# Tongji-MIC-Lab/TDVC

Hardware: AMD Instinct MI355X
Metric: 1080p P-frames/sec (encode + reconstruct, lambda=2048 config) (higher is better)
Workload: dtype f16; 1 GPU; 1x 1920x1080 (padded 1088x1920) 7-frame synthetic GOP (seed 1234), batch 1, P-frames coded in GOP order; gop=7, batch=1, parallelism=gop-sharded x1, weights=closed-form filler (no checkpoint ships)

## Files before the change

include/tdvc_hip.h:

```cpp
#ifndef TDVC_HIP_H
#define TDVC_HIP_H

#include <stdint.h>

#ifdef __cplusplus
extern "C" {
#endif

#define TDVC_OK 0
#define TDVC_EINVAL (-1)
#define TDVC_ENOSUP (-2)

typedef struct {
  void* p;
  int32_t N, H, W, C;
  int64_t sn;
  int32_t sp;
  int32_t dtype;
} tdvc_fmap;

enum { TDVC_F16 = 0, TDVC_F32 = 1 };
enum { TDVC_ACT_NONE = 0, TDVC_ACT_RELU = 1, TDVC_ACT_LRELU = 2, TDVC_ACT_CLAMP01 = 3, TDVC_ACT_SIGMOID = 4 };
enum { TDVC_GDN_NONE = 0, TDVC_GDN_FWD = 1, TDVC_GDN_INV = 2 };
enum { TDVC_OUT_NHWC = 0,
       TDVC_OUT_SHUFFLE2 = 1,
       TDVC_OUT_NCHW_F32 = 2 };

#define TDVC_MAX_TAPS 49

typedef struct {
  tdvc_fmap x;
  tdvc_fmap y;
  const void* w;
  const float* bias;
  int32_t cout;
  int32_t ntaps;
  int8_t tap_dy[TDVC_MAX_TAPS], tap_dx[TDVC_MAX_TAPS];
  int32_t kh, kw, stride, pad;
  int32_t ck;
  int32_t square_input;
  int32_t gdn;
  tdvc_fmap aux;
  int32_t act; float slope;
  int32_t round_before_act;
  tdvc_fmap res;
  tdvc_fmap res2;
  int32_t out_mode;
  int32_t s2d;
  int32_t bcast_T;
  float bcast_slope;
  float* chan_sum;
  tdvc_fmap flow;
} tdvc_conv_desc;

int tdvc_abi_version(void);
const char* tdvc_last_error(void);
int tdvc_prepare_device(void);
const char* tdvc_last_conv_kernel(void);

int tdvc_set_predicate(const int* flag);
int tdvc_last_launch_predicated(void);
#define TDVC_MAX_PREDICATE_IMAGES 4
int tdvc_set_predicate_images(const int* flags, int n);
int tdvc_frame_changed(const tdvc_fmap* cur, tdvc_fmap* cache, int* flag, void* stream);
int tdvc_frames_changed(const tdvc_fmap* cur, tdvc_fmap* cache, int* flags, unsigned force_mask, void* stream);


int tdvc_conv_plan(int cin, int kh, int kw, int stride);
int64_t tdvc_conv_packed_bytes(int cout, int cin, int ntaps, int ck);
int tdvc_pack_conv_weights(const float* w_oihw, int cout, int cin_real, int cin, int kh, int kw,
                           int ntaps, const int8_t* tap_dy, const int8_t* tap_dx, int ck, uint16_t* dst);
int tdvc_conv2d(const tdvc_conv_desc* d, void* stream);
int tdvc_conv_chan_sum_rows(const tdvc_conv_desc* d);
int tdvc_conv_flow_supported(const tdvc_conv_desc* d);
const char* tdvc_conv_select(const tdvc_conv_desc* d);
int tdvc_conv2d_f32(const tdvc_conv_desc* d, void* stream);

typedef struct {
  tdvc_fmap x, y;
  const void* w;
  const float* bias;
  int32_t act1; float slope1;
  int32_t act2; float slope2;
  int32_t add_input;
  tdvc_fmap res2;
} tdvc_conv_pair_desc;
int64_t tdvc_conv_pair_packed_bytes(void);
int tdvc_pack_conv_pair_weights(const float* w1_oihw, const float* w2_oihw, uint16_t* dst);
int tdvc_conv_pair_supported(const tdvc_conv_pair_desc* d);
int tdvc_conv_pair(const tdvc_conv_pair_desc* d, void* stream);

typedef struct {
  tdvc_fmap s, a, y;
  int32_t nslices;
  int32_t slice_stride;
  const void* wt;
  const float* bias_t;
  const void* w3;
  const float* bias3;
  float slope;
} tdvc_lf_tail_desc;
int tdvc_lf_tail_supported(const tdvc_lf_tail_desc* d);
int tdvc_lf_tail(const tdvc_lf_tail_desc* d, void* stream);

typedef struct {
  tdvc_fmap x, om, y;
  const void* w;
  const float* bias;
  int32_t groups;
  int32_t act; float slope; int32_t round_before_act;
  void* x_planar;
} tdvc_dcn_desc;
int tdvc_dcn_fused(const tdvc_dcn_desc* d, void* stream);

int tdvc_dcn_v2_forward_f32(const float* input, const float* weight, const float* bias,
                            const float* offset, const float* mask, float* output,
                            int B, int C, int H, int W, int Cout,
                            int kh, int kw, int sh, int sw, int ph, int pw, int dh, int dw,
                            int deformable_group, void* stream);
int tdvc_dcn_v2_backward_f32(const float* input, const float* weight, const float* bias,
                             const float* offset, const float* mask, const float* grad_output,
                             float* grad_input, float* grad_offset, float* grad_mask,
                             float* grad_weight, float* grad_bias, float* columns,
                             int B, int C, int H, int W, int Cout,
                             int kh, int kw, int sh, int sw, int ph, int pw, int dh, int dw,
                             int deformable_group, void* stream);

int tdvc_nchw_to_fmap(const float* src, int C, const tdvc_fmap* y, void* stream);
int tdvc_fmap_to_nchw(const tdvc_fmap* x, int C, float* dst, void* stream);
int tdvc_scale_act_res(const tdvc_fmap* a, const float* gate, int act, float slope,
                       const tdvc_fmap* r, float r_sign, const tdvc_fmap* y, const tdvc_fmap* y2, void* stream);
int tdvc_scale_act_res3(const tdvc_fmap* a, const float* gate, int act, float slope, const tdvc_fmap* r, float r_sign,
                        const tdvc_fmap* y, const tdvc_fmap* b, float b_sign, const tdvc_fmap* y3, void* stream);
int tdvc_add_flow(const tdvc_fmap* off, const tdvc_fmap* flow, void* stream);
int tdvc_bcast_add_act(const tdvc_fmap* x, const tdvc_fmap* b, int T, float slope, void* stream);

int tdvc_channel_sum(const tdvc_fmap* x, float* partial, int nblocks, void* stream);
int tdvc_se_gate(const float* partial, int nblocks, float inv_count, int N, int C, int Cmid,
                 const float* w1, const float* b1, const float* w2, const float* b2,
                 float* gate, void* stream);

int tdvc_upsample2x(const tdvc_fmap* x, const tdvc_fmap* y, void* stream);
int tdvc_avgpool2(const tdvc_fmap* x, const tdvc_fmap* y, void* stream);
int tdvc_avgpool2_pyramid(const tdvc_fmap* xa, const tdvc_fmap* xb, const tdvc_fmap* ya, const tdvc_fmap* yb, void* stream);
int tdvc_spynet_level_input(const tdvc_fmap* ref, const tdvc_fmap* supp, const tdvc_fmap* flow_lo,
                            const tdvc_fmap* flow_up, const tdvc_fmap* cat8, void* stream);
int tdvc_resize_bilinear(const tdvc_fmap* x, const tdvc_fmap* y, const float* chscale, void* stream);

int64_t tdvc_avgpool_k_work_floats(int N, int hp, int wp, int C, int scale);
int tdvc_avgpool_k(const tdvc_fmap* x, int scale, float* pooled, int hp, int wp, float* work, int64_t work_floats, void* stream);
int tdvc_patch_match(const float* pin, const float* pref, int N, int hp, int wp, int C,
                     int32_t* idx, void* stream);
int tdvc_match_gather(const tdvc_fmap* fin, const tdvc_fmap* fref, const int32_t* idx, int scale,
                      int hp, int wp, const tdvc_fmap* cat, void* stream);

int tdvc_eb_forward(const tdvc_fmap* z, const float* params, const tdvc_fmap* noise,
                    const tdvc_fmap* z_hat, double* bits_out, float* partial, int partial_cap, void* stream);
int tdvc_gc_forward(const tdvc_fmap* y, const tdvc_fmap* gp, const tdvc_fmap* noise,
                    double* bits_out, float* partial, int partial_cap, void* stream);
int tdvc_quantize(const tdvc_fmap* y, const tdvc_fmap* noise, const tdvc_fmap* y_hat, void* stream);

int64_t tdvc_rans_encode(const int32_t* symbols, const int32_t* indexes, int64_t n,
                         const int32_t* cdfs, int32_t cdf_stride, const int32_t* cdf_sizes,
                         const int32_t* offsets, uint8_t* out, int64_t cap);
int tdvc_rans_decode(const uint8_t* data, int64_t nbytes, const int32_t* indexes, int64_t n,
                     const int32_t* cdfs, int32_t cdf_stride, const int32_t* cdf_sizes,
                     const int32_t* offsets, int32_t* symbols_out);

void* tdvc_rans_decoder_create(const uint8_t* data, int64_t nbytes);
int tdvc_rans_decoder_decode(void* handle, const int32_t* indexes, int64_t n, const int32_t* cdfs,
                             int32_t cdf_stride, const int32_t* cdf_sizes, const int32_t* offsets,
                             int32_t* symbols_out);
void tdvc_rans_decoder_destroy(void* handle);

int64_t tdvc_rans_encode_lanes(const int32_t* symbols, const int32_t* indexes, int64_t npos, int M, int L,
                               const int32_t* cdfs, int32_t cdf_stride, const int32_t* cdf_sizes,
                               const int32_t* offsets, uint8_t* out, int64_t cap);
int tdvc_rans_decode_lanes(const uint8_t* data, int64_t nbytes, const int32_t* indexes, int64_t npos, int M,
                           const int32_t* cdfs, int32_t cdf_stride, const int32_t* cdf_sizes,
                           const int32_t* offsets, int32_t* symbols_out);

int tdvc_pmf_to_quantized_cdf(const float* pmf, int n, int precision, int32_t* cdf_out);

int tdvc_ar_gather_batch(const tdvc_fmap* y_hat, const tdvc_fmap* params, const int32_t* pos, int npos,
                         const tdvc_fmap* x1, const tdvc_fmap* pc, void* stream);
int tdvc_ar_quantize_batch(const tdvc_fmap* y, const tdvc_fmap* gp, const int32_t* pos, int npos, const float* scale_table, int ntable,
                           const int32_t* symbols_in, const tdvc_fmap* y_hat, int32_t* symbols, int32_t* indexes, int64_t cbase, void* stream);
int tdvc_ar_indexes_batch(const tdvc_fmap* gp, const int32_t* pos, int npos, int B, const float* scale_table, int ntable,
                          int M, int H, int W, int32_t* indexes, int64_t cbase, void* stream);
typedef struct tdvc_cdf_tables {
  const int32_t *cdfs, *sizes, *offsets;
  int32_t stride, ncdfs;
} tdvc_cdf_tables;
typedef struct tdvc_cdf_tables_dev {
  const uint16_t* cdf16;
  const int32_t *starts, *sizes, *offsets;
  int32_t n16, ncdfs;
} tdvc_cdf_tables_dev;
typedef struct tdvc_ar_loop {
  tdvc_fmap y_hat, params;
  tdvc_fmap x1, pc, gp;
  const tdvc_conv_desc* convs;
  int32_t nconvs;
  const int32_t* pos_dev;
  const int32_t* step_sizes;
  int32_t nsteps;
  const float* scale_table;
  int32_t ntable;
  int32_t *idx_dev, *sym_dev;
} tdvc_ar_loop;
int tdvc_ar_wavefront_batch(const tdvc_ar_loop* loop, const tdvc_fmap* y, const uint8_t* const* data, const int64_t* nbytes,
                            const tdvc_cdf_tables* tables, void* stream);
int tdvc_ar_decode_serial_batch(const tdvc_ar_loop* loop, const uint8_t* const* data, const int64_t* nbytes, const tdvc_cdf_tables* tables,
                                void* stream);
int64_t tdvc_ar_lanes_state_bytes(int L);
int64_t tdvc_ar_lanes_batch_layout(const int64_t* nbytes, int B, int L, uint32_t* table_out);
int tdvc_ar_lanes_init_batch(const uint8_t* streams_dev, int64_t stream_bytes, const uint32_t* table_dev, int B, int L, uint32_t* state_dev, void* stream);
int tdvc_ar_decode_lanes_step_batch(const tdvc_fmap* gp, const int32_t* pos, int npos, const float* scale_table, int ntable,
                                    const uint8_t* streams_dev, int64_t stream_bytes, const uint32_t* table_dev, int L,
                                    const tdvc_cdf_tables_dev* tables, uint32_t* state_dev, const tdvc_fmap* y_hat,
                                    int32_t* symbols, int32_t* indexes, int64_t cbase, void* stream);
int tdvc_ar_wavefront_lanes_batch(const tdvc_ar_loop* loop, const uint8_t* const* data, const int64_t* nbytes, uint8_t* stream_dev,
                                  int64_t stream_cap, uint32_t* state_dev, const tdvc_cdf_tables_dev* tables, int32_t* bad_image, void* stream);
int64_t tdvc_ar_encode_lanes_scratch_words(int64_t npos, int M, int L);
int64_t tdvc_ar_encode_lanes_out_bytes(int64_t npos, int M, int L);
typedef struct tdvc_lanes_enc {
  const int32_t *symbols, *indexes;
  int32_t B, H, W, M;
// ... 118 lines not shown
```

tdvc_amd/_lib.py:

```python
from __future__ import annotations

import ctypes as C
import os

_HERE = os.path.dirname(os.path.abspath(__file__))
LIB_PATH = os.path.join(_HERE, "libtdvc_hip.so")

MAX_TAPS = 49
F16, F32 = 0, 1
ACT_NONE, ACT_RELU, ACT_LRELU, ACT_CLAMP01, ACT_SIGMOID = 0, 1, 2, 3, 4
GDN_NONE, GDN_FWD, GDN_INV = 0, 1, 2
OUT_NHWC, OUT_SHUFFLE2, OUT_NCHW_F32 = 0, 1, 2


class FMapDesc(C.Structure):
    _fields_ = [("p", C.c_void_p), ("N", C.c_int32), ("H", C.c_int32), ("W", C.c_int32), ("C", C.c_int32),
                ("sn", C.c_int64), ("sp", C.c_int32), ("dtype", C.c_int32)]


class ConvDesc(C.Structure):
    _fields_ = [("x", FMapDesc), ("y", FMapDesc), ("w", C.c_void_p), ("bias", C.c_void_p),
                ("cout", C.c_int32), ("ntaps", C.c_int32),
                ("tap_dy", C.c_int8 * MAX_TAPS), ("tap_dx", C.c_int8 * MAX_TAPS),
                ("kh", C.c_int32), ("kw", C.c_int32), ("stride", C.c_int32), ("pad", C.c_int32),
                ("ck", C.c_int32), ("square_input", C.c_int32), ("gdn", C.c_int32),
                ("aux", FMapDesc), ("act", C.c_int32), ("slope", C.c_float),
                ("round_before_act", C.c_int32), ("res", FMapDesc), ("res2", FMapDesc), ("out_mode", C.c_int32), ("s2d", C.c_int32),
                ("bcast_T", C.c_int32), ("bcast_slope", C.c_float), ("chan_sum", C.c_void_p), ("flow", FMapDesc)]


class DcnDesc(C.Structure):
    _fields_ = [("x", FMapDesc), ("om", FMapDesc), ("y", FMapDesc), ("w", C.c_void_p), ("bias", C.c_void_p),
                ("groups", C.c_int32), ("act", C.c_int32), ("slope", C.c_float), ("round_before_act", C.c_int32), ("x_planar", C.c_void_p)]


class ConvPairDesc(C.Structure):
    _fields_ = [("x", FMapDesc), ("y", FMapDesc), ("w", C.c_void_p), ("bias", C.c_void_p), ("act1", C.c_int32), ("slope1", C.c_float),
                ("act2", C.c_int32), ("slope2", C.c_float), ("add_input", C.c_int32), ("res2", FMapDesc)]


class LfTailDesc(C.Structure):
    _fields_ = [("s", FMapDesc), ("a", FMapDesc), ("y", FMapDesc), ("nslices", C.c_int32), ("slice_stride", C.c_int32),
                ("wt", C.c_void_p), ("bias_t", C.c_void_p), ("w3", C.c_void_p), ("bias3", C.c_void_p), ("slope", C.c_float)]


class WgradReduceJob(C.Structure):
    _fields_ = [("work", C.c_void_p), ("bwork", C.c_void_p), ("row_off", C.c_void_p), ("chan_off", C.c_void_p), ("tap_off", C.c_void_p),
                ("bias_index", C.c_void_p), ("dw", C.c_void_p), ("db", C.c_void_p), ("scale", C.c_float),
                ("nworkers", C.c_int32), ("cow", C.c_int32), ("ciw", C.c_int32), ("ntaps", C.c_int32), ("cout", C.c_int32), ("cin", C.c_int32),
                ("wblocks", C.c_int32), ("nblocks", C.c_int32)]


_P = C.c_void_p
_FM = C.POINTER(FMapDesc)


class CdfTablesDesc(C.Structure):
    _fields_ = [("cdfs", _P), ("sizes", _P), ("offsets", _P), ("stride", C.c_int32), ("ncdfs", C.c_int32)]


class CdfTablesDevDesc(C.Structure):
    _fields_ = [("cdf16", _P), ("starts", _P), ("sizes", _P), ("offsets", _P), ("n16", C.c_int32), ("ncdfs", C.c_int32)]


class ArLoopDesc(C.Structure):
    _fields_ = [("y_hat", FMapDesc), ("params", FMapDesc), ("x1", FMapDesc), ("pc", FMapDesc), ("gp", FMapDesc),
                ("convs", C.POINTER(ConvDesc)), ("nconvs", C.c_int32), ("pos_dev", _P), ("step_sizes", _P), ("nsteps", C.c_int32),
                ("scale_table", _P), ("ntable", C.c_int32), ("idx_dev", _P), ("sym_dev", _P)]


class LanesEncDesc(C.Structure):
    _fields_ = [("symbols", _P), ("indexes", _P), ("B", C.c_int32), ("H", C.c_int32), ("W", C.c_int32), ("M", C.c_int32), ("pos", _P),
                ("npos", C.c_int32), ("L", C.c_int32), ("scratch", _P), ("lane_words", C.c_int64), ("scratch_cap_words", C.c_int64),
                ("out", _P), ("out_stride", C.c_int64), ("out_cap", C.c_int64), ("info", _P)]


_LOOP, _CDF, _CDFD, _ENC = C.POINTER(ArLoopDesc), C.POINTER(CdfTablesDesc), C.POINTER(CdfTablesDevDesc), C.POINTER(LanesEncDesc)
_i, _f, _i64 = C.c_int, C.c_float, C.c_int64

SIGNATURES = {
    "tdvc_abi_version": (_i, []),
    "tdvc_conv_chan_sum_rows": (_i, [C.POINTER(ConvDesc)]),
    "tdvc_conv_select": (C.c_char_p, [C.POINTER(ConvDesc)]),
    "tdvc_conv_flow_supported": (_i, [C.POINTER(ConvDesc)]),
    "tdvc_scale_act_res3": (_i, [_FM, _P, _i, _f, _FM, _f, _FM, _FM, _f, _FM, _P]),
    "tdvc_avgpool2_pyramid": (_i, [_FM, _FM, _FM, _FM, _P]),
    "tdvc_last_error": (C.c_char_p, []),
    "tdvc_last_conv_kernel": (C.c_char_p, []),
    "tdvc_prepare_device": (_i, []),
    "tdvc_set_predicate": (_i, [_P]),
    "tdvc_set_predicate_images": (_i, [_P, _i]),
    "tdvc_last_launch_predicated": (_i, []),
    "tdvc_frame_changed": (_i, [_FM, _FM, _P, _P]),
    "tdvc_frames_changed": (_i, [_FM, _FM, _P, C.c_uint, _P]),
    "tdvc_conv_plan": (_i, [_i, _i, _i, _i]),
    "tdvc_conv_packed_bytes": (_i64, [_i, _i, _i, _i]),
    "tdvc_pack_conv_weights": (_i, [_P, _i, _i, _i, _i, _i, _i, _P, _P, _i, _P]),
    "tdvc_conv2d": (_i, [C.POINTER(ConvDesc), _P]),
    "tdvc_conv2d_f32": (_i, [C.POINTER(ConvDesc), _P]),
    "tdvc_pack_conv_weights_indexed": (_i, [_P] * 7 + [_i] * 4 + [_P, _P]),
    "tdvc_pack_conv_weights_indexed_f32": (_i, [_P] * 7 + [_i] * 4 + [_P, _P]),
    "tdvc_pack_job_blocks": (_i64, [_i, _i, _i, _i]),
    "tdvc_pack_conv_weights_batch": (_i, [_P, _P, _i, _i, _P]),
    "tdvc_act_backward": (_i, [_FM, _FM, _FM, _i, _f, _FM, _P]),
    "tdvc_pixel_unshuffle": (_i, [_FM, _FM, _P]),
    "tdvc_bias_grad_work_floats": (_i64, [_i, _i]),
    "tdvc_bias_grad": (_i, [_FM, _i, _P, _f, _P, _P, _i64, _P]),
    "tdvc_copy_cast": (_i, [_FM, _FM, _P]),
    "tdvc_clamp01_backward": (_i, [_FM, _FM, _P]),
    "tdvc_gate_backward_work_floats": (_i64, [_i, _i]),
    "tdvc_gate_backward": (_i, [_FM, _FM, _P, _FM, _P, _P, _i64, _P]),
    "tdvc_se_gate_backward": (_i, [_P, _i, _f, _i, _i, _i] + [_P] * 6 + [_f] + [_P] * 6),
    "tdvc_bcast_channel_add": (_i, [_FM, _P, _f, _P]),
    "tdvc_add_flow_backward": (_i, [_FM, _FM, _P]),
    "tdvc_bcast_add_act_backward": (_i, [_FM, _FM, _FM, _f, _P]),
    "tdvc_upsample2x_backward": (_i, [_FM, _FM, _P]),
    "tdvc_resize_bilinear_backward": (_i, [_FM, _FM, _P, _P]),
    "tdvc_spynet_level_input_backward": (_i, [_FM, _FM, _FM, _FM, _FM, _P]),
    "tdvc_sigmoid_f32": (_i, [_P, _P, _i64, _P]),
    "tdvc_sigmoid_backward_f32": (_i, [_P, _P, _i64, _P]),
    "tdvc_axpy_f32": (_i, [_P, _P, _f, _i64, _P]),
    "tdvc_match_gather_backward": (_i, [_FM, _FM, _P, _i, _i, _i, _FM, _FM, _FM, _P]),
    "tdvc_eb_backward": (_i, [_FM, _P, _FM, _f, _FM, _P, _P]),
    "tdvc_eb_pack": (_i, [_P, _P, _P, _i, _P]),
    "tdvc_eb_param_chain": (_i, [_P, _P, _P, _f, _i, _P]),
    "tdvc_eb_aux": (_i, [_P, _P, _f, _P, _P, _i, _P]),
    "tdvc_gc_backward": (_i, [_FM, _FM, _FM, _f, _FM, _FM, _P]),
    "tdvc_dcn_columns": (_i, [_FM, _FM, _i, _FM, _P]),
    "tdvc_ar_lanes_state_bytes": (_i64, [_i]),
    "tdvc_ar_gather_batch": (_i, [_FM, _FM, _P, _i, _FM, _FM, _P]),
    "tdvc_ar_quantize_batch": (_i, [_FM, _FM, _P, _i, _P, _i, _P, _FM, _P, _P, _i64, _P]),
    "tdvc_ar_indexes_batch": (_i, [_FM, _P, _i, _i, _P, _i, _i, _i, _i, _P, _i64, _P]),
    "tdvc_ar_wavefront_batch": (_i, [_LOOP, _FM, _P, _P, _CDF, _P]),
    "tdvc_ar_decode_serial_batch": (_i, [_LOOP, _P, _P, _CDF, _P]),
    "tdvc_ar_lanes_batch_layout": (_i64, [_P, _i, _i, _P]),
    "tdvc_ar_lanes_init_batch": (_i, [_P, _i64, _P, _i, _i, _P, _P]),
    "tdvc_ar_decode_lanes_step_batch": (_i, [_FM, _P, _i, _P, _i, _P, _i64, _P, _i, _CDFD, _P, _FM, _P, _P, _i64, _P]),
    "tdvc_ar_wavefront_lanes_batch": (_i, [_LOOP, _P, _P, _P, _i64, _P, _CDFD, C.POINTER(C.c_int32), _P]),
    "tdvc_ar_encode_lanes_scratch_words": (_i64, [_i64, _i, _i]),
    "tdvc_ar_encode_lanes_out_bytes": (_i64, [_i64, _i, _i]),
    "tdvc_ar_encode_lanes_batch": (_i, [_ENC, _CDFD, _P]),
    "tdvc_rans_encode_lanes_dev_ref": (_i, [_ENC, _CDF]),
    "tdvc_ar_last_loop_launches": (_i64, []),
    "tdvc_ssim_level_work_floats": (_i64, [_i] * 5),
    "tdvc_ssim_level": (_i, [_P, _P, _i, _i, _i, _i, _P, _i, _f, _f, _P, _P, _P, _i64, _P]),
    "tdvc_avgpool2_pad_f32": (_i, [_P, _i64, _i, _i, _P, _P]),
    "tdvc_ssim_level_backward": (_i, [_P, _P, _i, _i, _i, _i, _P, _i, _f, _f, _P, _P, _f, _P, _P, _P]),
    "tdvc_msssim_level_grads": (_i, [_P, _P, _P, _i, _i, _P, _P, _P, _P, _P]),
    "tdvc_dcn_col2im_work_floats": (_i64, [_i, _i, _i, _i]),
    "tdvc_dcn_col2im_tile": (_i, []),
    "tdvc_dcn_col2im": (_i, [_FM, _FM, _FM, _i, _P, _FM, _P, _i64, _P]),
    "tdvc_dcn_col2im_det": (_i, [_FM, _FM, _FM, _i, _P, _FM, _P, _i64, _P, _P, _P, _i, _P]),
    "tdvc_dcn_far_apply": (_i, [_P, _P, _P, _i, _P, _P]),
    "tdvc_conv_wgrad_work_floats": (_i64, [_i] * 6),
    "tdvc_conv_wgrad": (_i, [_FM, _FM] + [_i] * 6 + [_P] * 5 + [_i, _f, _P, _P, _i64, _P]),
    "tdvc_conv_wgrad_bias": (_i, [_FM, _FM] + [_i] * 6 + [_P] * 5 + [_i, _f, _P, _P, _P, _P, _i64, _P]),
    "tdvc_conv_wgrad_partials": (_i, [_FM, _FM] + [_i] * 6 + [_P] * 5 + [_i, _f, _P, _P, _P, _P, _i64, C.POINTER(WgradReduceJob), _P]),
    "tdvc_wgrad_reduce_batch": (_i, [_P, _P, _i, _i, _P]),
    "tdvc_gdn_backward": (_i, [_FM, _FM, _FM, _i, _FM, _FM, _P]),
    "tdvc_mul2_accumulate": (_i, [_FM, _FM, _FM, _P]),
    "tdvc_dcn_fused": (_i, [C.POINTER(DcnDesc), _P]),
    "tdvc_conv_pair_packed_bytes": (_i64, []),
    "tdvc_pack_conv_pair_weights": (_i, [_P, _P, _P]),
    "tdvc_conv_pair_supported": (_i, [C.POINTER(ConvPairDesc)]),
    "tdvc_conv_pair": (_i, [C.POINTER(ConvPairDesc), _P]),
    "tdvc_lf_tail_supported": (_i, [C.POINTER(LfTailDesc)]),
    "tdvc_lf_tail": (_i, [C.POINTER(LfTailDesc), _P]),
    "tdvc_dcn_v2_forward_f32": (_i, [_P] * 6 + [_i] * 14 + [_P]),
    "tdvc_dcn_v2_backward_f32": (_i, [_P] * 12 + [_i] * 14 + [_P]),
    "tdvc_nchw_to_fmap": (_i, [_P, _i, _FM, _P]),
    "tdvc_fmap_to_nchw": (_i, [_FM, _i, _P, _P]),
    "tdvc_scale_act_res": (_i, [_FM, _P, _i, _f, _FM, _f, _FM, _FM, _P]),
    "tdvc_add_flow": (_i, [_FM, _FM, _P]),
    "tdvc_bcast_add_act": (_i, [_FM, _FM, _i, _f, _P]),
    "tdvc_channel_sum": (_i, [_FM, _P, _i, _P]),
    "tdvc_se_gate": (_i, [_P, _i, _f, _i, _i, _i, _P, _P, _P, _P, _P, _P]),
    "tdvc_upsample2x": (_i, [_FM, _FM, _P]),
    "tdvc_avgpool2": (_i, [_FM, _FM, _P]),
    "tdvc_spynet_level_input": (_i, [_FM, _FM, _FM, _FM, _FM, _P]),
    "tdvc_resize_bilinear": (_i, [_FM, _FM, _P, _P]),
    "tdvc_avgpool_k_work_floats": (_i64, [_i, _i, _i, _i, _i]),
    "tdvc_avgpool_k": (_i, [_FM, _i, _P, _i, _i, _P, _i64, _P]),
    "tdvc_patch_match": (_i, [_P, _P, _i, _i, _i, _i, _P, _P]),
    "tdvc_match_gather": (_i, [_FM, _FM, _P, _i, _i, _i, _FM, _P]),
    "tdvc_eb_forward": (_i, [_FM, _P, _FM, _FM, _P, _P, _i, _P]),
    "tdvc_gc_forward": (_i, [_FM, _FM, _FM, _P, _P, _i, _P]),
    "tdvc_quantize": (_i, [_FM, _FM, _FM, _P]),
    "tdvc_rans_encode": (_i64, [_P, _P, _i64, _P, C.c_int32, _P, _P, _P, _i64]),
    "tdvc_rans_decode": (_i, [_P, _i64, _P, _i64, _P, C.c_int32, _P, _P, _P]),
    "tdvc_rans_encode_lanes": (_i64, [_P, _P, _i64, _i, _i, _P, C.c_int32, _P, _P, _P, _i64]),
    "tdvc_rans_decode_lanes": (_i, [_P, _i64, _P, _i64, _i, _P, C.c_int32, _P, _P, _P]),
    "tdvc_rans_decoder_create": (_P, [_P, _i64]),
    "tdvc_rans_decoder_decode": (_i, [_P, _P, _i64, _P, C.c_int32, _P, _P, _P]),
    "tdvc_rans_decoder_destroy": (None, [_P]),
    "tdvc_pmf_to_quantized_cdf": (_i, [_P, _i, _i, _P]),
    "tdvc_round_symbols": (_i, [_FM, _P, _P, _P]),
}

_lib = None


class TdvcHipError(RuntimeError):
    pass


class TdvcStreamError(TdvcHipError, ValueError):
    """a damaged y string met by a batched decoder: the message names the image of the call"""


def lib():
    global _lib
    if _lib is None:
        if not os.path.exists(LIB_PATH):
            raise TdvcHipError(
                f"{LIB_PATH} is missing: build it with `python -c 'import __graft_entry__ as g; g.build()'` "
                "(hipcc --offload-arch=gfx950).  tdvc_amd has no CPU fallback.")
        l = C.CDLL(LIB_PATH)
        for name, (res, args) in SIGNATURES.items():
            fn = getattr(l, name)
            fn.restype = res
            fn.argtypes = args
        _lib = l
    return _lib


def check(rc: int, what: str = ""):
    if rc != 0:
        msg = lib().tdvc_last_error().decode("utf-8", "replace")
        raise TdvcHipError(f"{what}: rc={rc}: {msg}")
```

tdvc_amd/autograd.py:

```python
from __future__ import annotations

import contextlib

import torch

from . import ops
from .ops import FM


LAZY_IDENTITY = True
BATCH_WGRAD_REDUCE = True


class MirrorPool:
    ARENA_BYTES = 1 << 30

    def __init__(self):
        self.free: dict = {}
        self.used: list = []
        self.arenas: list = []
        self.loose: list = []

    def _carve(self, like: torch.Tensor) -> torch.Tensor:
        nbytes = like.numel() * like.element_size()
# ... 47 lines not shown
        self.side = None
        self.pool: MirrorPool | None = None
        self.wbatch = ops.WgradBatch() if BATCH_WGRAD_REDUCE else None
        self.fused_aux = False
        self.touched: set = set()
        self.pending: dict = {}
        self.deferred: list = []
        self.gdn_items: list = []
        self._ev, self._side_raw = None, None

    def _mirror(self, t: torch.Tensor) -> torch.Tensor:
        key = t.data_ptr()
        g = self.gbuf.get(key)
        if g is None:
            g = self.pool.get(t) if self.pool is not None else torch.zeros_like(t)
            self.gbuf[key] = g
            self.keep.append(t)
        return g

    def _base(self, t: torch.Tensor) -> torch.Tensor:
        key = t.data_ptr()
        g = self._mirror(t)
        self.touched.add(key)
        p = self.pending.pop(key, None)
        if p is not None:
            pf, src = p
            accumulate(FM(g, pf.off, pf.N, pf.C, pf.sn), src)
        return g

    def add_identity(self, fm: FM, src: FM):
        key = fm.t.data_ptr()
        if not LAZY_IDENTITY or key in self.touched or key in self.pending or src.f32 or fm.f32 or src.C != fm.C:
            accumulate(self.grad(fm), src if src.C <= fm.C else src.ch(0, fm.C))
            return False
        self.pending[key] = (fm, src)
        return True

    def grad_for_write(self, fm: FM):
        key = fm.t.data_ptr()
        if not LAZY_IDENTITY or key in self.touched:
            return self.grad(fm), True, None
        p = self.pending.get(key)
        if p is not None and (p[0].off, p[0].N, p[0].C, p[0].sn) != (fm.off, fm.N, fm.C, fm.sn):
            return self.grad(fm), True, None
        self.pending.pop(key, None)
        self.touched.add(key)
        return FM(self._mirror(fm.t), fm.off, fm.N, fm.C, fm.sn), False, (p[1] if p is not None else None)

    def grad(self, fm: FM) -> FM:
        return FM(self._base(fm.t), fm.off, fm.N, fm.C, fm.sn)

    def grad_tensor(self, t: torch.Tensor) -> torch.Tensor:
        return self._base(t)

    def zeros_like(self, t: torch.Tensor) -> torch.Tensor:
        if self.pool is not None and t.is_contiguous() and t.dtype in (torch.float32, torch.float16):
            return self.pool.get(t.detach())
        return torch.zeros_like(t)

    def needs_grad(self, fm: FM) -> bool:
        return fm.t.data_ptr() not in self.nograd

    def mark_input(self, fm: FM):
        self.nograd.add(fm.t.data_ptr())

    def add(self, fn):
        self.nodes.append(fn)

    def defer(self, fn):
        self.deferred.append(fn)

    def off_path(self, fn, *tensors):
        if self.side is None:
            return fn()
        ev = self._ev
        if ev is None:
            ev = self._ev = torch.cuda.Event()
            self._side_raw = self.side.cuda_stream
        ev.record()
        self.side.wait_event(ev)
        self.keep.extend(tensors)
        ops.FORCE_STREAM, ops.FORCE_KEEP = self._side_raw, self.keep
        try:
            fn()
        finally:
            ops.FORCE_STREAM, ops.FORCE_KEEP = None, None

    def release(self):
        self.nodes.clear()
        self.deferred.clear()
        self.gbuf.clear()
        self.keep.clear()
        self.pending.clear()
        self.touched.clear()
        self.on_node_done = None
        self.touch_log = None
        self.pool = None

    def join(self):
        if self.wbatch is not None and self.wbatch.items:
            if self.side is not None:
                with torch.cuda.stream(self.side):
                    self.wbatch.flush()
            else:
                self.wbatch.flush()
        if self.side is not None:
            torch.cuda.current_stream().wait_stream(self.side)

    def touch(self, *params):
        if self.touch_log is not None:
            for q in params:
                self.touch_log[id(q)] = self._cur

    @property
    def inv_scale(self) -> float:
        return 1.0 / self.loss_scale

    def backward(self):
        prev, ops._IN_BACKWARD = ops._IN_BACKWARD, True
        try:
            self.n_backward_nodes = len(self.nodes)
            for k, fn in enumerate(reversed(self.nodes)):
                self._cur = k
                fn()
                if self.on_node_done is not None:
                    self.on_node_done(k)
            self.join()
            self._cur = self.n_backward_nodes
            for fn in self.deferred:
                fn()
        finally:
            self.join()
            ops._IN_BACKWARD = prev
            self._cur = -1
        self.nodes.clear()
        self.deferred.clear()


def param_grad(p: torch.Tensor) -> torch.Tensor:
    if p.grad is None:
        p.grad = torch.zeros_like(p, dtype=torch.float32)
    t = ops.TAPE
    if t is not None:
        t.touch(p)
    return p.grad


@contextlib.contextmanager
def record(loss_scale: float = 1.0, side_stream=None, pool: MirrorPool | None = None):
    tape = Tape(loss_scale)
    tape.side = side_stream
    tape.pool = pool
    prev, ops.TAPE = ops.TAPE, tape
    try:
        yield tape
    finally:
        ops.TAPE = prev


def accumulate(dst: FM, src: FM, sign: float = 1.0):
    ops.scale_act_res(dst, dst, res=src, res_sign=sign)


def record_conv(tape: Tape, x: FM, pc, y, act, slope, res, res2, gdn, aux, square, nchw_out):
    if gdn != ops.GDN_NONE:
        return record_gdn(tape, x, pc, y, res, gdn)
    assert not square
    assert not (act not in (ops.ACT_NONE,) and res2 is not None), "autograd: activation + two residuals is not on the path"
    weight, bias = pc.param_w, pc.param_b

    def bwd():
        if nchw_out is not None:
            gdt = torch.float32 if x.f32 else torch.float16
            g = ops.from_nchw(tape.grad_tensor(nchw_out), Cpad=ops.pad8(pc.cout), dtype=gdt)
            yv = ops.from_nchw(nchw_out, Cpad=ops.pad8(pc.cout), dtype=gdt)
        else:
            g, yv = tape.grad(y), y
        held = False
        if res is not None and tape.needs_grad(res):
            held |= tape.add_identity(res, g)
        if res2 is not None and tape.needs_grad(res2):
            held |= tape.add_identity(res2, g)
        if x.f32:
            if not g.f32:
                g = ops.copy_cast(g, FM.empty(g.N, g.H, g.W, g.C, dtype=torch.float32, device=g.t.device))
                held = False
        elif g.f32:
            g = ops.copy_cast(g, FM.empty(g.N, g.H, g.W, ops.pad8(g.C), device=g.t.device))
            held = False
        fresh = (lambda: FM.empty(g.N, g.H, g.W, g.C, dtype=g.t.dtype, device=g.t.device)) if held else (lambda: None)
        if act in (ops.ACT_RELU, ops.ACT_LRELU):
            g = ops.act_backward(g, yv, act, slope, res=res, out=fresh())
        elif act == ops.ACT_CLAMP01:
            g = ops.clamp01_backward(g, yv) if not held else ops.clamp01_backward(ops.copy_cast(g, fresh()), yv)
        elif act != ops.ACT_NONE:
            raise NotImplementedError(f"autograd: activation {act}")
        gq = ops.pixel_unshuffle(g) if pc.shuffle else g
        tape.off_path(lambda: ops.conv_wgrad(pc, gq, x, param_grad(weight).view(-1), scale=tape.inv_scale,
                                             db=param_grad(bias) if bias is not None else None,
                                             defer=tape.wbatch),
                      gq.t, x.t)
        if tape.needs_grad(x):
            gx, acc, extra = tape.grad_for_write(x)
            ops.conv_dgrad(pc, gq, gx, accumulate=acc, extra=extra)

    tape.add(bwd)


def record_scale_act_res(tape: Tape, a: FM, out: FM, gate, act, slope, res, res_sign, out2):
    def bwd():
        g = tape.grad(out)
        if out2 is not None:
            accumulate(g, tape.grad(out2))
        if res is not None and tape.needs_grad(res):
            if res_sign == 1.0:
                tape.add_identity(res, g)
            else:
                accumulate(tape.grad(res), g, res_sign)
        if act in (ops.ACT_RELU, ops.ACT_LRELU):
            g = ops.act_backward(g, out, act, slope, res=res, out=FM.empty(g.N, g.H, g.W, g.C, dtype=g.t.dtype, device=g.t.device))
        elif act != ops.ACT_NONE:
            raise NotImplementedError(f"autograd: scale_act_res with activation {act}")
        if gate is not None:
            ops.gate_backward(g, a, gate, tape.grad(a) if tape.needs_grad(a) else None, tape.grad_tensor(gate))
        elif tape.needs_grad(a):
            tape.add_identity(a, g)

    tape.add(bwd)


def record_se_gate(tape: Tape, x: FM, p, partial, nblocks, gate):
    params = p.params

    def bwd():
        dgate = tape.grad_tensor(gate)
        grads = [param_grad(q) for q in params]
        dmean = ops.se_gate_backward(p, partial, nblocks, x.H * x.W, gate, dgate, tape.inv_scale, grads)
        if tape.needs_grad(x):
            ops.bcast_channel_add(tape.grad(x), dmean, 1.0 / (x.H * x.W))

    tape.add(bwd)


def record_cast(tape: Tape, x: FM, out: FM):
    def bwd():
        if tape.needs_grad(x):
            accumulate(tape.grad(x), tape.grad(out))

    tape.add(bwd)


def record_clone(tape: Tape, x: FM, out: FM):
    def bwd():
        if tape.needs_grad(x):
            tape.add_identity(x, tape.grad(out))

    tape.add(bwd)


def record_add_flow(tape: Tape, off: FM, flow: FM):
    tape.add(lambda: ops.add_flow_backward(tape.grad(off), tape.grad(flow)))


def record_bcast_add_act(tape: Tape, x: FM, b: FM, slope):
    tape.add(lambda: ops.bcast_add_act_backward(tape.grad(x), x, tape.grad(b), slope))


def record_upsample2x(tape: Tape, x: FM, out: FM):
    def bwd():
        if tape.needs_grad(x):
            ops.upsample2x_backward(tape.grad(out), tape.grad(x))

    tape.add(bwd)


def record_resize_bilinear(tape: Tape, x: FM, out: FM, chscale):
    def bwd():
        if tape.needs_grad(x):
            ops.resize_bilinear_backward(tape.grad(out), tape.grad(x), chscale)

    tape.add(bwd)


def record_spynet_level_input(tape: Tape, supp: FM, flow_lo, flow_up: FM, cat8: FM):
    tape.add(lambda: ops.spynet_level_input_backward(supp, flow_up, tape.grad(cat8), tape.grad(flow_up),
                                                     tape.grad(flow_lo) if flow_lo is not None else None))


def record_dcn_fused(tape: Tape, x: FM, om: FM, pc, out: FM, groups, act, slope):
    weight, bias = pc.param_w, pc.param_b

    def bwd():
        g = tape.grad(out)
        if act in (ops.ACT_RELU, ops.ACT_LRELU):
            g = ops.act_backward(g, out, act, slope)
        if x.f32 and not g.f32:
            g = ops.copy_cast(g, FM.empty(g.N, g.H, g.W, g.C, dtype=torch.float32, device=g.t.device))
        cpc = ops.dcn_column_conv(pc, groups)
        col = ops.dcn_columns(x, om, groups)
        ops.conv_wgrad(cpc, g, col, param_grad(weight).view(-1), scale=tape.inv_scale, db=param_grad(bias))
        dcol = ops.conv_dgrad(cpc, g, col, accumulate=False)
        dx32 = ops.dcn_col2im(x, om, dcol, groups, tape.grad(om))
        if tape.needs_grad(x):
            accumulate(tape.grad(x), dx32)

    tape.add(bwd)


def record_match_gather(tape: Tape, fin: FM, fref: FM, idx, scale, cat: FM):
    tape.add(lambda: ops.match_gather_backward(fin, fref, idx, scale, tape.grad(cat), tape.grad(fin), tape.grad(fref)))
# ... 58 lines not shown
```

tdvc_amd/csrc/conv_mfma.hip:

```cpp
#include "conv_common.h"

using convk::ConvParams;

namespace {

constexpr int TH = 8, TW = 32;

template <int CK8, int MT, int STRIDE, bool LEAN = false>
__global__ __launch_bounds__(256, LEAN ? 3 : 1) void conv_mfma_kernel(const ConvParams p) {
  extern __shared__ __attribute__((aligned(16))) unsigned char smem[];
  constexpr int CK = CK8 * 8;
  constexpr int PS = (CK8 == 1) ? 16 : CK * 2 + 16;
  int* tapoff = reinterpret_cast<int*>(smem);
  unsigned char* tile = smem + 256;

  const int tid = threadIdx.x, lane = tid & 63, wave = tid >> 6;
  const int hh = lane >> 5, r = lane & 31;
  const int tile_id = convk::block_tile(p);
  const int tx = tile_id % p.tiles_x, ty = tile_id / p.tiles_x;
  const int cb = blockIdx.y, n = blockIdx.z;

  const int TIH = (TH - 1) * STRIDE + p.kh;
  const int TIW = (TW - 1) * STRIDE + p.kw;
  const int HALFW = (TIW + 1) >> 1;
// ... 34 lines not shown

    const half_t* wp[MT];
#pragma unroll
    for (int mt = 0; mt < MT; ++mt)
      wp[mt] = p.w + ((((long)(cb * MT + mt) * p.nchunks + ch) * p.steps) * 64 + lane) * 8;

    if constexpr (CK8 == 1) {
      for (int s = 0; s < p.steps; ++s) {
        int tap = 2 * s + hh;
        tap = tap < p.ntaps ? tap : p.ntaps - 1;
        const int toff = tapoff[tap];
        half8 a[MT], b[2];
#pragma unroll
        for (int mt = 0; mt < MT; ++mt) { a[mt] = *reinterpret_cast<const half8*>(wp[mt]); wp[mt] += 512; }
#pragma unroll
        for (int nt = 0; nt < 2; ++nt) b[nt] = *reinterpret_cast<const half8*>(tile + base[nt] + toff);
#pragma unroll
        for (int mt = 0; mt < MT; ++mt)
#pragma unroll
          for (int nt = 0; nt < 2; ++nt)
            acc[mt][nt] = __builtin_amdgcn_mfma_f32_32x32x16_f16(a[mt], b[nt], acc[mt][nt], 0, 0, 0);
      }
    } else {
      for (int tap = 0; tap < p.ntaps; ++tap) {
        const int toff = tapoff[tap] + hh * 16;
#pragma unroll
        for (int s2 = 0; s2 < CK8 / 2; ++s2) {
          half8 a[MT], b[2];
#pragma unroll
          for (int mt = 0; mt < MT; ++mt) { a[mt] = *reinterpret_cast<const half8*>(wp[mt]); wp[mt] += 512; }
#pragma unroll
          for (int nt = 0; nt < 2; ++nt)
            b[nt] = *reinterpret_cast<const half8*>(tile + base[nt] + toff + s2 * 32);
#pragma unroll
          for (int mt = 0; mt < MT; ++mt)
#pragma unroll
            for (int nt = 0; nt < 2; ++nt)
              acc[mt][nt] = __builtin_amdgcn_mfma_f32_32x32x16_f16(a[mt], b[nt], acc[mt][nt], 0, 0, 0);
        }
      }
    }
  }

  if constexpr (MT == 2 && LEAN) {
    __syncthreads();
    convk::epilogue_simple_rows<2, false, 2>(p, acc, p.bias + cb * 64, tile + wave * (32 * 144), n, cb * 64,
                                             ty * TH + wave * 2, tx * TW, lane, false);
    return;
  } else if constexpr (MT == 2) {
    if (p.simple) {
      __syncthreads();
      convk::epilogue_simple_rows<2, false, 1>(p, acc, p.bias + cb * 64, tile + wave * (32 * 144), n, cb * 64,
                                               ty * TH + wave * 2, tx * TW, lane, false);
      return;
    }
  }
  convk::epilogue_regs(p, acc, n, ty * TH + wave * 2, tx * TW + r, cb * MT, hh);
}

template <int CK8, int MT, int STRIDE>
int launch(const ConvParams& p, dim3 grid, size_t lds, hipStream_t st) {
  if constexpr (MT == 2) {
    if (p.simple == 2) {
      hipLaunchKernelGGL((conv_mfma_kernel<CK8, MT, STRIDE, true>), grid, dim3(256), lds, st, p);
      return tdvc_launch_status("tdvc_conv2d");
    }
  }
  hipLaunchKernelGGL((conv_mfma_kernel<CK8, MT, STRIDE, false>), grid, dim3(256), lds, st, p);
  return tdvc_launch_status("tdvc_conv2d");
}

template <int CK8, int MT>
int launch_s(const ConvParams& p, int stride, dim3 grid, size_t lds, hipStream_t st) {
  return stride == 1 ? launch<CK8, MT, 1>(p, grid, lds, st) : launch<CK8, MT, 2>(p, grid, lds, st);
}

template <int CK8>
int launch_m(const ConvParams& p, int mt, int stride, dim3 grid, size_t lds, hipStream_t st) {
  return mt == 1 ? launch_s<CK8, 1>(p, stride, grid, lds, st) : launch_s<CK8, 2>(p, stride, grid, lds, st);
}

inline int lds_bytes(int ck, int kh, int kw, int stride) {
  const int ps = (ck == 8) ? 16 : ck * 2 + 16;
  const int tih = (TH - 1) * stride + kh, tiw = (TW - 1) * stride + kw;
  const int tiwp = stride == 2 ? 2 * ((tiw + 1) >> 1) : tiw;
  return 256 + tih * tiwp * ps;
}

inline int cout_tiles(int cout) { return cout <= 32 ? 1 : 2 * ((cout + 63) / 64); }

}

extern "C" int tdvc_conv_plan(int cin, int kh, int kw, int stride) {
  if (cin <= 0 || (cin % 8) != 0 || kh < 1 || kw < 1 || kh > 7 || kw > 7 || (stride != 1 && stride != 2)) {
    tdvc_set_error("tdvc_conv_plan: unsupported geometry cin=%d k=%dx%d stride=%d", cin, kh, kw, stride);
    return TDVC_EINVAL;
  }
  const int cands[4] = {64, 32, 16, 8};
  for (int i = 0; i < 4; ++i) {
    const int ck = cands[i];
    if (ck > cin && ck != 8) {
      if (cin % ck != 0 && cin < ck) continue;
    }
    if (lds_bytes(ck, kh, kw, stride) <= 64 * 1024) return ck;
  }
  tdvc_set_error("tdvc_conv_plan: no LDS plan for k=%dx%d stride=%d", kh, kw, stride);
  return TDVC_EINVAL;
}

extern "C" int64_t tdvc_conv_packed_bytes(int cout, int cin, int ntaps, int ck) {
  if (cout <= 0 || cin <= 0 || ntaps <= 0 || ntaps > TDVC_MAX_TAPS || (ck != 8 && ck != 16 && ck != 32 && ck != 64)) return TDVC_EINVAL;
  const int ck8 = ck / 8;
  const int64_t nchunks = (cin + ck - 1) / ck;
  const int64_t steps = (ntaps * ck8 + 1) / 2;
  return (int64_t)cout_tiles(cout) * nchunks * steps * 64 * 8 * 2;
}

extern "C" int tdvc_pack_conv_weights(const float* w, int cout, int cin_real, int cin, int kh, int kw,
                                      int ntaps, const int8_t* tap_dy, const int8_t* tap_dx, int ck, uint16_t* dst) {
  TDVC_CHECK(w && dst && tap_dy && tap_dx, "tdvc_pack_conv_weights: null pointer");
  TDVC_CHECK(tdvc_conv_packed_bytes(cout, cin, ntaps, ck) > 0, "tdvc_pack_conv_weights: bad geometry");
  TDVC_CHECK(cin_real <= cin, "tdvc_pack_conv_weights: cin_real > cin");
  const int ck8 = ck / 8;
  const int nchunks = (cin + ck - 1) / ck;
  const int steps = (ntaps * ck8 + 1) / 2;
  const int tiles = cout_tiles(cout);
  half_t* out = reinterpret_cast<half_t*>(dst);
  for (int t = 0; t < tiles; ++t)
    for (int ch = 0; ch < nchunks; ++ch)
      for (int s = 0; s < steps; ++s)
        for (int lane = 0; lane < 64; ++lane) {
          const int r = lane & 31, h = lane >> 5;
          const int co = t * 32 + r;
          const int kc = 2 * s + h;
          half_t* o = out + ((((int64_t)t * nchunks + ch) * steps + s) * 64 + lane) * 8;
          for (int j = 0; j < 8; ++j) {
            float v = 0.f;
            if (kc < ntaps * ck8 && co < cout) {
              const int tap = kc / ck8, c8 = kc % ck8;
              const int ci = ch * ck + c8 * 8 + j;
              const int dy = tap_dy[tap], dx = tap_dx[tap];
              if (ci < cin_real && dy >= 0 && dy < kh && dx >= 0 && dx < kw)
                v = w[(((int64_t)co * cin_real + ci) * kh + dy) * kw + dx];
            }
            o[j] = (half_t)v;
          }
        }
  return TDVC_OK;
}

int conv_direct_lds_bytes(const tdvc_conv_desc* d) { return lds_bytes(d->ck, d->kh, d->kw, d->stride); }
int conv_cout_tiles(int cout) { return cout_tiles(cout); }

int launch_conv_direct(const ConvParams& p, int ck8, int stride, int N, hipStream_t st) {
  const int tiles = cout_tiles(p.cout), mt = tiles == 1 ? 1 : 2;
  const int lds = lds_bytes(ck8 * 8, p.kh, p.kw, stride);
  const dim3 grid(p.tiles_x * ((p.Ho + TH - 1) / TH), tiles / mt, N);
  const size_t lds_v1 = (p.simple && lds < 256 + 4 * 32 * 144) ? 256 + 4 * 32 * 144 : lds;
  switch (ck8) {
    case 1: return launch_m<1>(p, mt, stride, grid, lds_v1, st);
    case 2: return launch_m<2>(p, mt, stride, grid, lds_v1, st);
    case 4: return launch_m<4>(p, mt, stride, grid, lds_v1, st);
    default: return launch_m<8>(p, mt, stride, grid, lds_v1, st);
  }
}
```

Before: 54.12 frames/s.

## Add persistent tap-column MFMA kernel for 7x7 64->32 stride-1 convolutions

Adds a specialized persistent kernel for 7x7, 64-input, 32-output, stride-1 convs (typical of optical-flow SpyNet-style layers). It reuses each loaded input column across the seven vertical taps in registers and double-buffers the input tile and the weight fragments in LDS, walking tiles in an XCD-aware order. The kernel is chosen by a tile-count heuristic between 8- and 16-row-per-wave variants, and is disabled while autograd recording is active. The new path adds code complexity and uses large LDS (launch_big_lds) with one block per CU.

```diff
diff --git a/include/tdvc_hip.h b/include/tdvc_hip.h
--- a/include/tdvc_hip.h
+++ b/include/tdvc_hip.h
@@ -74,6 +74,9 @@
 int tdvc_conv_chan_sum_rows(const tdvc_conv_desc* d);
 int tdvc_conv_flow_supported(const tdvc_conv_desc* d);
 const char* tdvc_conv_select(const tdvc_conv_desc* d);
+void tdvc_debug_enable_conv_tapcol(int mask);
+void tdvc_debug_set_conv_tapcol_min_pixels(long min_pixels);
+int tdvc_debug_conv_direct_last_form(void);
 int tdvc_conv2d_f32(const tdvc_conv_desc* d, void* stream);
 
 typedef struct {
diff --git a/tdvc_amd/_lib.py b/tdvc_amd/_lib.py
--- a/tdvc_amd/_lib.py
+++ b/tdvc_amd/_lib.py
@@ -83,6 +83,9 @@
     "tdvc_conv_chan_sum_rows": (_i, [C.POINTER(ConvDesc)]),
     "tdvc_conv_select": (C.c_char_p, [C.POINTER(ConvDesc)]),
     "tdvc_conv_flow_supported": (_i, [C.POINTER(ConvDesc)]),
+    "tdvc_debug_enable_conv_tapcol": (None, [_i]),
+    "tdvc_debug_set_conv_tapcol_min_pixels": (None, [C.c_long]),
+    "tdvc_debug_conv_direct_last_form": (_i, []),
     "tdvc_scale_act_res3": (_i, [_FM, _P, _i, _f, _FM, _f, _FM, _FM, _f, _FM, _P]),
     "tdvc_avgpool2_pyramid": (_i, [_FM, _FM, _FM, _FM, _P]),
     "tdvc_last_error": (C.c_char_p, []),
diff --git a/tdvc_amd/autograd.py b/tdvc_amd/autograd.py
--- a/tdvc_amd/autograd.py
+++ b/tdvc_amd/autograd.py
@@ -223,10 +223,13 @@
     tape.side = side_stream
     tape.pool = pool
     prev, ops.TAPE = ops.TAPE, tape
+    ops.L.lib().tdvc_debug_enable_conv_tapcol(0)
     try:
         yield tape
     finally:
         ops.TAPE = prev
+        if prev is None:
+            ops.L.lib().tdvc_debug_enable_conv_tapcol(3)
 
 
 def accumulate(dst: FM, src: FM, sign: float = 1.0):
diff --git a/tdvc_amd/csrc/conv_mfma.hip b/tdvc_amd/csrc/conv_mfma.hip
--- a/tdvc_amd/csrc/conv_mfma.hip
+++ b/tdvc_amd/csrc/conv_mfma.hip
@@ -210,7 +210,14 @@
 int conv_direct_lds_bytes(const tdvc_conv_desc* d) { return lds_bytes(d->ck, d->kh, d->kw, d->stride); }
 int conv_cout_tiles(int cout) { return cout_tiles(cout); }
 
+int conv_tapcol_form(const ConvParams& p, int ck8, int stride, int N);
+int launch_conv_tapcol(int form, const ConvParams& p, int N, hipStream_t st);
+void conv_direct_note_form(int form);
+
 int launch_conv_direct(const ConvParams& p, int ck8, int stride, int N, hipStream_t st) {
+  const int form = conv_tapcol_form(p, ck8, stride, N);
+  conv_direct_note_form(form);
+  if (form) return launch_conv_tapcol(form, p, N, st);
   const int tiles = cout_tiles(p.cout), mt = tiles == 1 ? 1 : 2;
   const int lds = lds_bytes(ck8 * 8, p.kh, p.kw, stride);
   const dim3 grid(p.tiles_x * ((p.Ho + TH - 1) / TH), tiles / mt, N);
diff --git a/tdvc_amd/csrc/conv_tapcol.hip b/tdvc_amd/csrc/conv_tapcol.hip
--- /dev/null
+++ b/tdvc_amd/csrc/conv_tapcol.hip
@@ -0,0 +1,189 @@
+#include <stdlib.h>
+
+#include "conv_common.h"
+
+using convk::ConvParams;
+
+namespace {
+
+typedef unsigned u32x4 __attribute__((ext_vector_type(4)));
+
+constexpr int TC_NTHR = 512, TC_TW = 32, TC_K = 7;
+constexpr int TC_IW = TC_TW + TC_K - 1;
+constexpr int TC_PS = 48;
+constexpr int TC_KSTEPS = 4;
+constexpr int TC_FRAG = 512;
+constexpr int TC_ABUF = TC_K * 1024;
+constexpr int TC_STEPS = 98;
+
+template <int RW>
+struct Geo {
+  static constexpr int TH = 8 * RW, IH = TH + TC_K - 1;
+  static constexpr int ITEMS = IH * TC_IW * 2;
+  static constexpr int PER_THR = (ITEMS + TC_NTHR - 1) / TC_NTHR;
+  static constexpr int BUF = IH * TC_IW * TC_PS;
+  static constexpr int LDS = 2 * BUF + 2 * TC_ABUF;
+};
+
+struct TapcolExtra {
+  int ntiles, tiles_x, tiles_per_img;
+};
+
+template <int RW>
+__global__ __launch_bounds__(TC_NTHR, 1) void conv_tapcol_kernel(const ConvParams p, const TapcolExtra e) {
+  using G = Geo<RW>;
+  extern __shared__ __attribute__((aligned(16))) unsigned char smem[];
+  const int tid = threadIdx.x, lane = tid & 63;
+  const int wave = __builtin_amdgcn_readfirstlane(tid >> 6);
+  const int hh = lane >> 5, r = lane & 31;
+
+  int first, stride, my_tiles;
+  convk::xcd_tile_walk(e.ntiles, first, stride, my_tiles);
+  if (my_tiles <= 0) return;
+  const int nstages = my_tiles * TC_KSTEPS;
+
+  u32x4 sreg[G::PER_THR];
+  unsigned okmask = 0u;
+  auto issue = [&](int s) {
+    const int tile_i = convk::walk_tile(p, e.ntiles, first, stride, s >> 2), ks = s & 3;
+    const int n = tile_i / e.tiles_per_img, rem = tile_i - n * e.tiles_per_img;
+    const int ty = rem / e.tiles_x, tx = rem - ty * e.tiles_x;
+    const half_t* xn = p.x + (long)n * p.x_sn + ks * 16;
+    const int iy0 = ty * G::TH - 3, ix0 = tx * TC_TW - 3;
+    unsigned m = 0u;
+#pragma unroll
+    for (int u = 0; u < G::PER_THR; ++u) {
+      const int idx = tid + u * TC_NTHR;
+      const int pix = idx >> 1, c2 = idx & 1;
+      const int rr = pix / TC_IW, cc = pix - rr * TC_IW;
+      const int iy = iy0 + rr, ix = ix0 + cc;
+      const bool ok = (int)(idx < G::ITEMS) & (int)(iy >= 0) & (int)(iy < p.H) & (int)(ix >= 0) & (int)(ix < p.W);
+      const half_t* src = xn + ((long)(ok ? iy : 0) * p.W + (ok ? ix : 0)) * p.x_sp + c2 * 8;
+      sreg[u] = *reinterpret_cast<const u32x4*>(src);
+      m |= (ok ? 1u : 0u) << u;
+    }
+    okmask = m;
+  };
+  auto publish = [&](int buf) {
+    unsigned char* tile = smem + buf * G::BUF;
+#pragma unroll
+    for (int u = 0; u < G::PER_THR; ++u) {
+      const int idx = tid + u * TC_NTHR;
+      const int pix = idx >> 1, c2 = idx & 1;
+      const u32x4 z = {0u, 0u, 0u, 0u};
+      const u32x4 val = ((okmask >> u) & 1u) ? sreg[u] : z;
+      if (idx < G::ITEMS) *reinterpret_cast<u32x4*>(tile + pix * TC_PS + c2 * 16) = val;
+    }
+  };
+
+  unsigned char* abuf = smem + 2 * G::BUF;
+  const bool amover = tid < TC_K * 64;
+  const half_t* wl = p.w + (long)(tid >> 6) * (2 * TC_K * TC_FRAG) + lane * 8;
+  u32x4 areg = {0u, 0u, 0u, 0u};
+  auto load_a = [&](int ks, int dx) {
+    if (amover) areg = *reinterpret_cast<const u32x4*>(wl + (long)((ks >> 1) * TC_STEPS + (ks & 1) + 2 * dx) * TC_FRAG);
+  };
+  auto write_a = [&](int par) {
+    if (amover) *reinterpret_cast<u32x4*>(abuf + par * TC_ABUF + tid * 16) = areg;
+  };
+
+  const int boff = ((wave * RW) * TC_IW + r) * TC_PS + hh * 16;
+
+  f32x16 acc[1][RW];
+  convk::zero_acc(acc);
+
+  issue(0);
+  load_a(0, 0);
+  write_a(0);
+  load_a(0, 1);
+  publish(0);
+  __syncthreads();
+
+#pragma unroll 1
+  for (int s = 0; s < nstages; ++s) {
+    const int ks = s & 3;
+    const bool more = s + 1 < nstages;
+    const unsigned char* bp = smem + (s & 1) * G::BUF + boff;
+    constexpr int NJ = RW + TC_K - 1, NT = TC_K * NJ;
+    auto read_b = [&](int t) { return *reinterpret_cast<const half8*>(bp + ((t % NJ) * TC_IW + t / NJ) * TC_PS); };
+    half8 b[3];
+    b[0] = read_b(0);
+    b[1] = read_b(1);
+#pragma unroll
+    for (int dx = 0; dx < TC_K; ++dx) {
+      const int par = (s + dx) & 1;
+      write_a(par ^ 1);
+      if (dx + 2 < TC_K) load_a(ks, dx + 2);
+      else load_a((ks + 1) & 3, dx + 2 - TC_K);
+      if (dx == 0) issue(more ? s + 1 : s);
+      half8 a_cur[TC_K];
+#pragma unroll
+      for (int dy = 0; dy < TC_K; ++dy) a_cur[dy] = *reinterpret_cast<const half8*>(abuf + par * TC_ABUF + (dy * 64 + lane) * 16);
+      __builtin_amdgcn_sched_barrier(0);
+#pragma unroll
+      for (int j = 0; j < NJ; ++j) {
+        const int t = dx * NJ + j;
+        if (t + 2 < NT) b[(t + 2) % 3] = read_b(t + 2);
+#pragma unroll
+        for (int dy = 0; dy < TC_K; ++dy)
+          if (j - dy >= 0 && j - dy < RW)
+            acc[0][j - dy] = __builtin_amdgcn_mfma_f32_32x32x16_f16(a_cur[dy], b[t % 3], acc[0][j - dy], 0, 0, 0);
+        __builtin_amdgcn_sched_barrier(0);
+      }
+      if (dx + 1 < TC_K) __syncthreads();
+    }
+    if (more) publish((s + 1) & 1);
+    if (ks == TC_KSTEPS - 1) {
+      const int tile_i = convk::walk_tile(p, e.ntiles, first, stride, s >> 2);
+      const int n = tile_i / e.tiles_per_img, rem = tile_i - n * e.tiles_per_img;
+      const int ty = rem / e.tiles_x, tx = rem - ty * e.tiles_x;
+      convk::epilogue_regs(p, acc, n, ty * G::TH + wave * RW, tx * TC_TW + r, 0, hh);
+      convk::zero_acc(acc);
+    }
+    __syncthreads();
+  }
+}
+
+int g_tapcol_mask = 3;
+constexpr long TC_MIN_PIXELS = 136L * 240;
+long g_tapcol_min_pixels = TC_MIN_PIXELS;
+constexpr int TC_TALL_MIN_TILES = 256;
+thread_local int g_direct_last_form = 0;
+
+template <int RW>
+int launch_tapcol(const ConvParams& p, int N, hipStream_t st) {
+  using G = Geo<RW>;
+  TapcolExtra e;
+  e.tiles_x = (p.Wo + TC_TW - 1) / TC_TW;
+  e.tiles_per_img = e.tiles_x * ((p.Ho + G::TH - 1) / G::TH);
+  e.ntiles = N * e.tiles_per_img;
+  const int grid = e.ntiles < 256 ? e.ntiles : 256;
+  return convk::launch_big_lds<&conv_tapcol_kernel<RW>, ConvParams, TapcolExtra>("tdvc_conv2d(tapcol)", 160 * 1024, dim3(grid), dim3(TC_NTHR), G::LDS, st, p, e);
+}
+
+}
+
+extern "C" void tdvc_debug_enable_conv_tapcol(int mask) { g_tapcol_mask = mask; }
+extern "C" void tdvc_debug_set_conv_tapcol_min_pixels(long v) { g_tapcol_min_pixels = v < 0 ? TC_MIN_PIXELS : v; }
+extern "C" int tdvc_debug_conv_direct_last_form(void) { return g_direct_last_form; }
+void conv_direct_note_form(int form) { g_direct_last_form = form; }
+
+int conv_tapcol_form(const ConvParams& p, int ck8, int stride, int N) {
+  static const bool env_off = getenv("TDVC_CONV_V1") != nullptr || getenv("TDVC_CONV_NO_TAPCOL") != nullptr;
+  if (env_off || !(g_tapcol_mask & 3)) return 0;
+  if (!(ck8 == 4 && stride == 1 && p.in_stride == 1 && p.kh == TC_K && p.kw == TC_K && p.pad == 3 && p.ntaps == TC_K * TC_K && p.Cin == 64 &&
+        p.nchunks == 2 && p.steps == TC_STEPS && p.cout == 32 && p.out_mode == TDVC_OUT_NHWC && !p.y.f32 && !p.res.p && !p.res2.p && !p.gdn &&
+        !p.square && !p.round16 && !p.s2d && !p.simple && !p.bcast_T && !p.csum && !p.flow.p &&
+        (p.act == TDVC_ACT_NONE || p.act == TDVC_ACT_RELU)))
+    return 0;
+  for (int t = 0; t < TC_K * TC_K; ++t)
+    if (p.tap_dy[t] != t / TC_K || p.tap_dx[t] != t % TC_K) return 0;
+  if ((long)N * p.Ho * p.Wo < g_tapcol_min_pixels) return 0;
+  const long tall_tiles = (long)N * ((p.Wo + TC_TW - 1) / TC_TW) * ((p.Ho + 31) / 32);
+  const int want = tall_tiles >= TC_TALL_MIN_TILES ? 1 : 2;
+  return (g_tapcol_mask & want) ? want : (3 - want);
+}
+
+int launch_conv_tapcol(int form, const ConvParams& p, int N, hipStream_t st) {
+  return form == 1 ? launch_tapcol<4>(p, N, st) : launch_tapcol<2>(p, N, st);
+}
```

Result: no change. 54.14 frames/s, median of 5 (+0.0%).
